# StuLiu/RegDA

Measured on AMD Instinct MI355X. Metric: src+tgt 512x512 image-pairs/sec (SSL step), higher is better.
Workload: dtype bf16; 1 GPU; st.regda.2potsdam SSL step, resnet101 DeepLabV2(PPM), batch 8+8 512x512 per GPU, online EMA teacher; global_batch=8, parallelism=dp1

## Files before the change

include/rgda_hip.h:

```cpp
#ifndef RGDA_HIP_H
#define RGDA_HIP_H

#include <stddef.h>
#include <stdint.h>

#ifdef __cplusplus
extern "C" {
#endif

#define RGDA_ABI_VERSION 10
#define RGDA_STAT_REPLICAS 8
#define RGDA_STAT_FRAC_FWD 26
#define RGDA_STAT_FRAC_BWD 40
typedef int64_t rgda_stat_t;
#define RGDA_LAYOUT_TILE 64

typedef void* rgda_stream_t;

enum rgda_status {
    RGDA_OK = 0,
    RGDA_ERR_ARG = -1,
    RGDA_ERR_WORKSPACE = -2,
    RGDA_ERR_LAUNCH = -3,
    RGDA_ERR_UNSUPPORTED = -4
// ... 237 lines not shown
int rgda_classifier_bwd(const void* hidden, int ldh, const float* w, const float* glogits,
                        void* dhidden, int lddh, float* dw, float* db, int N, int HW, int C,
                        int ncls, void* ws, size_t ws_bytes, rgda_stream_t stream);


int rgda_sumsq(const float* g, int64_t n, float* out, float* ws, rgda_stream_t stream);

int rgda_sgd_step(float* p, const float* g, float* v, float* shadow, void* p_bf16, void* shadow_bf16,
                  const float* gnorm_sq, const float* lr_dev, int64_t n, float momentum,
                  float weight_decay, float max_norm, float gscale, float ema_decay,
                  int first_step, rgda_stream_t stream);

size_t rgda_stem_wgrad_workspace(int N, int H, int W);
int rgda_stem_wgrad(const float* img, const void* dy, int lddy, float* dw, void* ws, size_t ws_bytes, int N, int H,
                    int W, int Ho, int Wo, rgda_stream_t stream);

int rgda_weight_transpose_bf16(const float* w, void* wt, int Co, int T, int Ci, rgda_stream_t stream);
int rgda_weight_transpose_batched(const int64_t* table, int n, int64_t total_blocks, rgda_stream_t stream);
int rgda_cast_bf16(const float* src, void* dst, int64_t n, rgda_stream_t stream);
int rgda_cast_f32(const void* src_bf16, float* dst, int64_t n, rgda_stream_t stream);
int rgda_ddp_accumulate_bf16(const void* recv, int world, void* out, int64_t shard_elems, rgda_stream_t stream);

typedef void* rgda_comm_t;
#define RGDA_COMM_ID_BYTES 128
#define RGDA_COMM_F32 0
#define RGDA_COMM_BF16 1
#define RGDA_COMM_I64 2
#define RGDA_COMM_F64 3
int rgda_comm_unique_id(void* id_128_bytes);
int rgda_comm_init(const void* id_128_bytes, int rank, int world, rgda_comm_t* comm);
// ... 185 lines not shown
```

regda_amd/csrc/common.h:

```cpp
#pragma once
#include <hip/hip_runtime.h>
#include <stdint.h>

#include "../../include/rgda_hip.h"

#define RGDA_CHECK_LAUNCH()                                   \
    do {                                                      \
        if (hipGetLastError() != hipSuccess) return RGDA_ERR_LAUNCH; \
    } while (0)

typedef unsigned short bf16_t;
typedef __attribute__((ext_vector_type(8))) __bf16 bf16x8;
typedef __attribute__((ext_vector_type(8))) unsigned short u16x8;
typedef __attribute__((ext_vector_type(4))) unsigned short u16x4;
typedef __attribute__((ext_vector_type(4))) short s16x4;
typedef __attribute__((ext_vector_type(16))) float f32x16;
typedef __attribute__((ext_vector_type(4))) float f32x4;

typedef __attribute__((ext_vector_type(2))) __bf16 bf16x2_t;
typedef __attribute__((ext_vector_type(2))) float f32x2_t;
static __device__ __forceinline__ float bf2f(bf16_t h) { return __uint_as_float(((unsigned)h) << 16); }
static __device__ __forceinline__ unsigned pack2bf(float lo, float hi) {
    f32x2_t v = {lo, hi};
    bf16x2_t b = __builtin_convertvector(v, bf16x2_t);
// ... 117 lines not shown
            const float unb = (b.rows_per_group > 1) ? (float)b.rows_per_group / (float)(b.rows_per_group - 1) : 1.f;
            float rm = b.rm ? b.rm[c] : 0.f, rv = b.rm ? b.rv[c] : 0.f;
            for (int g = 0; g < b.groups; ++g) {
                float gm, gv, gi;
                stat_moments(b.stats + (size_t)g * NREP * 2 * C, C, c, invM, b.eps, gm, gv, gi);
                if (b.mi) { b.mi[(size_t)g * 2 * C + c] = gm; b.mi[(size_t)g * 2 * C + C + c] = gi; }
                rm = (1.f - b.mom) * rm + b.mom * gm;
                rv = (1.f - b.mom) * rv + b.mom * gv * unb;
            }
            if (b.rm) { b.rm[c] = rm; b.rv[c] = rv; }
            if (c == 0 && b.nbt) *b.nbt += b.groups;
        }
    }
}

#include <stdlib.h>
#ifdef RGDA_TUNING
#define TUNE_ENV(name) getenv(name)
#else
#define TUNE_ENV(name) ((const char*)nullptr)
#endif
static inline hipStream_t to_stream(rgda_stream_t s) { return (hipStream_t)s; }
static inline int zero_bytes(void* p, size_t bytes, rgda_stream_t stream) {
    if (!((uintptr_t)p & 15)) return rgda_fill_zero(p, bytes, stream);
    return hipMemsetAsync(p, 0, bytes, (hipStream_t)stream) == hipSuccess ? RGDA_OK : RGDA_ERR_LAUNCH;
}
static inline int cdiv(long long a, long long b) { return (int)((a + b - 1) / b); }

#include <type_traits>
#define RGDA_MIN_CLASSES 6
// ... 17 lines not shown
```

regda_amd/csrc/conv_kernels.hip:

```cpp
#include <stdio.h>
#include <stdlib.h>
#include <string.h>

#include "common.h"
#include <type_traits>
#include <vector>

struct ConvArgs {
    const bf16_t* x;
    const bf16_t* w;
    bf16_t* y;
    const bf16_t* res;
    rgda_stat_t* stats;
    int ldx, ldy, ldres;
    int N, H, W, Cin, Ho, Wo, Cout, KH, KW, stride, pad, dil, mode;
    int M;
    int tiles_c, tiles_p;
    int rows_per_group;
    int howo_shift, wo_shift;
    unsigned long long* dbg;
    int tpw;
    int skip;
    const unsigned char* res_mask;
    const bf16_t* bn_y;
// ... 1775 lines not shown
    if (Ho != (H + 6 - 7) / 2 + 1 || Wo != (W + 6 - 7) / 2 + 1) return RGDA_ERR_ARG;
    if (Wo % 64) return RGDA_ERR_UNSUPPORTED;
    if ((long long)3 * H * W >= (1ll << 28)) return RGDA_ERR_UNSUPPORTED;
    if (((uintptr_t)ws & 15) || ws_bytes < rgda_stem_wgrad_workspace(N, H, W)) return RGDA_ERR_WORKSPACE;
    const int rpw = stem_wgrad_rows(N, Ho, Wo);
    const long long blocks = (long long)N * (Ho / rpw) * (Wo / 64);
    if (blocks > 0x7fffffffLL || (long long)N * Ho * Wo > 0x7fffffffLL) return RGDA_ERR_ARG;
    hipStream_t st = to_stream(stream);
    stem_wgrad_kernel<<<(int)blocks, 256, 0, st>>>(img, (const bf16_t*)dy, lddy, (float*)ws, H, W, Ho, Wo, rpw);
    RGDA_CHECK_LAUNCH();
    stem_wgrad_reduce_kernel<<<cdiv(64 * 147, 32), 256, 0, st>>>((const float*)ws, (int)blocks, dw);
    RGDA_CHECK_LAUNCH();
    return RGDA_OK;
}

extern "C" int rgda_stem_conv(const float* img, const void* wgt, void* y, int ldy, rgda_stat_t* stats, int stat_groups,
                              int N, int H, int W, int Ho, int Wo, rgda_stream_t stream) {
    return stem_conv_launch(img, wgt, y, ldy, stats, stat_groups, nullptr, N, H, W, Ho, Wo, stream);
}

extern "C" int rgda_stem_conv_bneval(const float* img, const void* wgt, void* y, int ldy, const float* running_mean,
                                     const float* running_var, const float* gamma, const float* beta, float eps, int relu,
                                     int N, int H, int W, int Ho, int Wo, rgda_stream_t stream) {
    BnEvalFuse e = {running_mean, running_var, gamma, beta, eps, relu};
    return stem_conv_launch(img, wgt, y, ldy, nullptr, 1, &e, N, H, W, Ho, Wo, stream);
}

struct WgradArgs {
    const bf16_t* x;
    const bf16_t* dy;
// ... 698 lines not shown
```

regda_amd/csrc/norm_kernels.hip:

```cpp
#include <stdlib.h>
#include "common.h"

struct RowLayout {
    int vpr;
    int vpb;
    int rpb;
};
static RowLayout row_layout(int C) {
    RowLayout L;
    L.vpr = C / 8;
    int v = 1;
    while (v < L.vpr && v < 256) v <<= 1;
    L.vpb = v;
    L.rpb = 256 / v;
    return L;
}

static int reduce_rows_per_block(long long M, const RowLayout& L) {
    int ny = cdiv(L.vpr, L.vpb);
    long long want = 512 / ny;
    if (const char* e = TUNE_ENV("RGDA_RED_WANT")) want = atoi(e) / ny;
    if (want < 1) want = 1;
    long long rows = (M + want - 1) / want;
    long long minrows = (long long)L.rpb * 4;
// ... 379 lines not shown
                }
                if (nscale) {
                    const float* ns = nscale + (r / rpi) * C + cg;
#pragma unroll
                    for (int e = 0; e < 8; ++e) gf[e] *= ns[e];
                }
#pragma unroll
                for (int e = 0; e < 8; ++e) { s[e] += gf[e]; q[e] += gf[e] * ((xf[e] - mean[e]) * istd[e]); }
            }
        }
    }
    rgda_stat_t* rep = sums + (size_t)((blockIdx.x + blockIdx.y * gridDim.x) & (NREP - 1)) * 2 * C;
    block_reduce_atomic(s, q, cvl, rl, vpb, rpb, cg, cok, rep, rep + C, lds, RGDA_STAT_FRAC_BWD);
}

extern "C" int rgda_bn_bwd_reduce(const void* g, int ldg, const void* y, int ldy, const uint8_t* relu_mask,
                                  const void* x, int ldx, const float* mi, const float* nscale, int rows_per_image,
                                  rgda_stat_t* sums, int64_t M, int C, int relu, const float* gamma, const float* beta,
                                  int groups, rgda_stream_t stream) {
    if (!g || !x || !mi || !sums || (relu == 1 && !y && !relu_mask) || M <= 0 || C <= 0 || (C & 7) || (ldg & 7) || (ldx & 7)) return RGDA_ERR_ARG;
    if (relu < 0 || relu > 2 || (relu == 2 && (!gamma || !beta))) return RGDA_ERR_ARG;
    if (groups < 1 || (M % groups)) return RGDA_ERR_ARG;
    hipStream_t st = to_stream(stream);
    RowLayout L = row_layout(C);
    if (L.vpb > 16) { L.vpb = 16; L.rpb = 16; }
    if (const char* e = TUNE_ENV("RGDA_RED_VPB")) { int v = atoi(e); if (v < L.vpb) { L.vpb = v; L.rpb = 256 / v; } }
    const long long Mg = M / groups;
    int rows_per_block = reduce_rows_per_block(Mg * groups, L);
    if (rows_per_block > Mg) rows_per_block = (int)((Mg + L.rpb - 1) / L.rpb * L.rpb);
    int bpg = cdiv(Mg, rows_per_block);
    dim3 grid(bpg * groups, cdiv(L.vpr, L.vpb));
    if (relu == 2)
        bn_bwd_reduce_kernel<true><<<grid, 256, 0, st>>>((const bf16_t*)g, ldg, (const bf16_t*)y, ldy, relu_mask, (const bf16_t*)x, ldx,
                                                         mi, nscale, rows_per_image, sums, Mg, C, relu, L.vpb, L.rpb,
                                                         rows_per_block, bpg, gamma, beta);
    else
        bn_bwd_reduce_kernel<false><<<grid, 256, 0, st>>>((const bf16_t*)g, ldg, (const bf16_t*)y, ldy, relu_mask, (const bf16_t*)x, ldx,
                                                          mi, nscale, rows_per_image, sums, Mg, C, relu, L.vpb, L.rpb,
                                                          rows_per_block, bpg, gamma, beta);
    RGDA_CHECK_LAUNCH();
    return RGDA_OK;
}

template <bool FROM_X>
__global__ void __launch_bounds__(256) bn_bwd_apply_kernel(const bf16_t* __restrict__ g, int ldg,
                                                           const bf16_t* __restrict__ y, int ldy,
// ... 6 lines not shown
                                                           float* dbeta, long long M, int C, int relu, int vpb, int rpb,
                                                           int rows_per_block, int bpg, const float* __restrict__ beta,
                                                           bf16_t* __restrict__ act_out, int ldact) {
    const int cvl = threadIdx.x % vpb, rl = threadIdx.x / vpb;
    const int cg = (blockIdx.y * vpb + cvl) * 8;
    const int grp = blockIdx.x / bpg, chunk = blockIdx.x % bpg;
    mi += (size_t)grp * 2 * C;
    sums += (size_t)grp * NREP * 2 * C;
    extern __shared__ __attribute__((aligned(16))) float sk_dyn[];
    const int nch = vpb * 8;
    float* const sk0 = sk_dyn;
    const float invM = 1.f / (float)M;
    for (int c = threadIdx.x; c < vpb * 8; c += 256) {
        const int cc = blockIdx.y * vpb * 8 + c;
        if (cc < C) {
            const float t1 = (float)stat_total(sums, C, cc, 0, RGDA_STAT_FRAC_BWD);
            const float t2 = (float)stat_total(sums, C, cc, 1, RGDA_STAT_FRAC_BWD);
            const float is = mi[C + cc];
            sk0[0 * nch + c] = mi[cc];
            sk0[1 * nch + c] = is;
            sk0[2 * nch + c] = gamma[cc] * is;
            sk0[3 * nch + c] = t1 * invM;
            sk0[4 * nch + c] = t2 * invM;
            if constexpr (FROM_X) {
                float fsc, fsh;
                bn_scale_shift(mi[cc], is, gamma[cc], beta[cc], fsc, fsh);
                sk0[5 * nch + c] = fsh;
            }
            if (chunk == 0 && grp == 0 && dgamma) {
                const int groups = gridDim.x / bpg;
                float dg = t2, db = t1;
                for (int g2 = 1; g2 < groups; ++g2) {
                    dg += (float)stat_total(sums + (size_t)g2 * NREP * 2 * C, C, cc, 1, RGDA_STAT_FRAC_BWD);
                    db += (float)stat_total(sums + (size_t)g2 * NREP * 2 * C, C, cc, 0, RGDA_STAT_FRAC_BWD);
                }
                atomicAdd(dgamma + cc, dg);
                atomicAdd(dbeta + cc, db);
            }
        }
    }
    __syncthreads();
    if (cg >= C) return;
    float mean[8], istd[8], k0[8], k1[8], k2[8], fsh[8];
#pragma unroll
    for (int e = 0; e < 8; ++e) {
        mean[e] = sk0[0 * nch + cvl * 8 + e];
        istd[e] = sk0[1 * nch + cvl * 8 + e];
        k0[e] = sk0[2 * nch + cvl * 8 + e];
        k1[e] = sk0[3 * nch + cvl * 8 + e];
        k2[e] = sk0[4 * nch + cvl * 8 + e];
        if constexpr (FROM_X) fsh[e] = sk0[5 * nch + cvl * 8 + e]; else fsh[e] = 0.f;
    }
// ... 37 lines not shown
                } else {
                    float yf[8];
                    cvt8(yv[u], yf);
#pragma unroll
                    for (int e = 0; e < 8; ++e) gf[e] = (yf[e] > 0.f) ? gf[e] : 0.f;
                }
            }
            if (nscale) {
                const float* ns = nscale + (r / rpi) * C + cg;
#pragma unroll
                for (int e = 0; e < 8; ++e) gf[e] *= ns[e];
            }
            if (gmask) store8(gmask + r * ldgm + cg, gf);
            float o[8];
#pragma unroll
            for (int e = 0; e < 8; ++e) o[e] = k0[e] * (gf[e] - k1[e] - (xf[e] - mean[e]) * istd[e] * k2[e]);
            store8(dx + r * lddx + cg, o);
        }
    }
}

extern "C" int rgda_bn_bwd_apply(const void* g, int ldg, const void* y, int ldy, const uint8_t* relu_mask,
                                 const void* x, int ldx,
                                 const float* mi, const float* gamma, const float* nscale, int rows_per_image,
                                 const rgda_stat_t* sums, void* dx, int lddx, void* gmask, int ldgm, float* dgamma,
                                 float* dbeta, int64_t M, int C, int relu, const float* beta, void* act_out, int ldact,
                                 int groups, rgda_stream_t stream) {
    if (!g || !x || !mi || !gamma || !sums || !dx || (relu == 1 && !y && !relu_mask) || M <= 0 || C <= 0 || (C & 7)) return RGDA_ERR_ARG;
    if (relu < 0 || relu > 2 || (relu == 2 && !beta) || (act_out && (relu != 2 || (ldact & 7) || ldact < C))) return RGDA_ERR_ARG;
    if ((ldg & 7) || (ldx & 7) || (lddx & 7) || (gmask && (ldgm & 7)) || ((dgamma == nullptr) != (dbeta == nullptr)))
        return RGDA_ERR_ARG;
// ... 1115 lines not shown
```

regda_amd/models/Encoder.py:

```python
import collections
import contextlib
import math
from typing import NamedTuple

import torch
import torch.nn as nn

from .. import ops
from .. import plan

BF = torch.bfloat16
LAYERS = {'resnet101': (3, 4, 23, 3), 'resnet50': (3, 4, 6, 3)}
POOL_SCALES = (1, 2, 3, 6)
NREP = 8
LAYOUT_TILE = 64


def _layout_blocks(co, ci, taps):
    return -(-ci // LAYOUT_TILE) * -(-co // LAYOUT_TILE) * taps

ASPP_DILATIONS = (6, 12, 18, 24)
STEM_KP = 192


# ... 168 lines not shown
WGRAD_FLUSH_AFTER = ('layer2',)


class _Unit(NamedTuple):
    x: object
    c: object
    y: object
    mi: object
    dims: tuple
    nscale: object
    rmask: object

    @property
    def on_operand_path(self):
        return self.rmask is FROM_X


class _UnitBwd:
    sums = None
    presums = None
    wgrad = None


_NO_UNIT_BWD = _UnitBwd()


class _WgradQueue:

    def __init__(self):
        self.items, self.flop, self._apart = [], 0.0, None
# ... 135 lines not shown
        self.resnet_type = rt
        self.num_classes = int(cfg['num_classes'])
        self.device = torch.device('cuda', torch.cuda.current_device())
        self._build_params()
        self._init_weights()
        self._anchor = torch.zeros(1, device=self.device, requires_grad=True)
        self._drop_override = None
        self.wgrad_group_gflop = 500.0
        self.relu_sign_mask = 1
        self.factored_ppm = True
        self.group_small_convs = True
        self.small_bn = True
        self.bn_on_operand = True
        self.bn_operand_units = {'stem', 'bn1', 'bn2'}
        self.bn_operand_level = 2
        self._head_stream = None
        self._mat_cache = {}
        self._synced_version = -1
        self.sync_weights()

    def _build_params(self):
        dev = self.device
        entries, self.blocks, self._head_first = _param_entries(self.resnet_type, self.head_kind, self.num_classes)

        n_param = sum(_pad64(math.prod(s)) for _, k, s in entries if k in ('convw', 'vec'))
        n_buf = sum(_pad64(math.prod(s)) for _, k, s in entries if k == 'buf')
        n_nbt = sum(1 for _, k, _s in entries if k == 'nbt')
        self.flat_p = torch.zeros(n_param, device=dev)
        self.flat_g = torch.zeros(n_param, device=dev)
        self.flat_pb = torch.zeros(n_param, dtype=BF, device=dev)
# ... 576 lines not shown
                                     1, dx_res, csums, G, ce.y if (crelu == 1 and cmask is None) else None, ce.c, ce.mi, crelu,
                                     ce.nscale, cHo * cWo, relu_mask=cmask, res_mask=dx_res_mask,
                                     bn_gamma=None if cbn is None else cbn.gamma, bn_beta=None if cbn is None else cbn.beta)
                    T['unit_bwd'][ckey].sums = csums
                    fused = True
                except ValueError:
                    T['unit_bwd'][ckey].presums = csums
            if not fused:
                if conv_queue is not None:
                    conv_queue.append((dc, conv.wtb, dx, N, Ho, Wo, H, W, conv.k, conv.k, conv.stride, conv.pad, conv.dil, 1,
                                       dx_res, None, 1, dx_res_mask))
                else:
                    ops.conv2d(dc, conv.wtb, dx, N, Ho, Wo, H, W, conv.k, conv.k, conv.stride, conv.pad, conv.dil, 1,
                               dx_res, None, res_mask=dx_res_mask)
        return dx, gm

    def _stem_fwd(self, T, xs, Ng, H, W, H1, W1, main_stream):
        dev = self.device
        bn = self.bns['encoder.resnet.bn1']
        G = len(xs)
        N, M = Ng * G, Ng * G * H1 * W1
        y = torch.empty(M, 64, dtype=BF, device=dev)
        if T is None:
            for gi, xg in enumerate(xs):
                ops.stem_conv_bneval(xg, self.stem_wb, y[gi * Ng * H1 * W1:(gi + 1) * Ng * H1 * W1], bn.rm, bn.rv, bn.gamma,
                                     bn.beta, True, Ng, H, W, H1, W1)
            return y, None
        side = self._side_stream()
        plan.wait_event(side, plan.record_event(main_stream))
        with ops.use_stream(side):
# ... 290 lines not shown
        hh, ww = h, w
        for bi in range(len(self.blocks) - 1, -1, -1):
            p, inpl, planes, stride, dil, ds = self.blocks[bi]
            if dbg is not None:
                dbg[p] = _nchw(g, N, hh, ww)
                hh, ww = hh * stride, ww * stride
            below = (self.blocks[bi - 1][0] + '.3', True) if bi > 0 else None
            g = self._block_bwd(T, self.blocks[bi], g, below)
            self._progress(T, self._offset_of(p + '.conv1'))
            if bi > 0 and T['wgrads'].items:
                stage = p.split('.')[-2]
                if stage in WGRAD_FLUSH_AFTER and self.blocks[bi - 1][0].split('.')[-2] != stage:
                    self._flush_wgrads(T)
        self._flush_wgrads(T)
        idx, (N, H1, W1, H2, W2) = T['pool']
        ga0 = torch.empty(N * H1 * W1, 64, dtype=BF, device=dev)
        ops.maxpool_bwd(g, idx, ga0, N, H1, W1, 64, H2, W2)
        self._cbr_bwd(T, 'stem', C['encoder.resnet.conv1'], B['encoder.resnet.bn1'], ga0, True, stem=True)
        self._flush_wgrads(T)
        if T.get('mark') is not None:
            T['mark']('backward main chain done')
        if T.get('wgrad_stream') is not None:
            plan.wait_stream(T['main_stream'], T['wgrad_stream'])

    def attach_grads(self):
        for name, par in self._views.items():
            par.grad = self._gviews[name]

    def _prepare_grads(self):
        if any(par.grad is None for par in self._views.values()):
            self.flat_g.zero_()
            self.attach_grads()

# ... 52 lines not shown
```

regda_amd/ops.py:

```python
import ctypes

import torch

from ._lib import lib


MIN_CLASSES, MAX_CLASSES = 6, 16


def check_class_count(c, who='class_num'):
    if not MIN_CLASSES <= int(c) <= MAX_CLASSES:
        raise ValueError(f'{who}: {c} classes; the kernels serve {MIN_CLASSES} <= class_num <= {MAX_CLASSES}')


_LDS_LOSS_ROW, _LDS_PCL, _LDS_REFINE = 0, 1, 2


def check_step_shape(c, k, H, W, who='step'):
    check_class_count(c, who)
    L = lib()
    w = (int(W) + 15) // 16
    row, lim = L.size('rgda_class_lds', _LDS_LOSS_ROW, c, w, W), L.size('rgda_class_lds_limit', _LDS_LOSS_ROW)
    if row > lim:
        raise ValueError(f'{who}: {c} classes at {W}-pixel rows need {row} B of LDS in the fused upsample + loss row pass, '
# ... 667 lines not shown


def stem_conv_bneval(img, wb, y, rm, rv, gamma, beta, relu, N, H, W, Ho, Wo, eps=1e-5):
    lib().call('rgda_stem_conv_bneval', img.data_ptr(), wb.data_ptr(), y.data_ptr(), _ld(y), rm.data_ptr(), rv.data_ptr(),
               gamma.data_ptr(), beta.data_ptr(), eps, int(relu), N, H, W, Ho, Wo, _stream())


def stem_im2col(img, col, N, H, W, Ho, Wo):
    lib().call('rgda_stem_im2col', img.data_ptr(), col.data_ptr(), N, H, W, Ho, Wo, col.shape[1], _stream())


_STEM_WS = {}
_STEM_WS_OLD = []


def stem_wgrad(img, dy, dw, N, H, W, Ho, Wo):
    assert dw.is_contiguous() and dw.dtype == torch.float32 and dw.numel() == 64 * 147 and img.is_contiguous()
    L = lib()
    nbytes = L.size('rgda_stem_wgrad_workspace', N, H, W)
    if nbytes == 0:
        raise ValueError('rgda_stem_wgrad: geometry not served (Wo % 64 != 0): use stem_im2col + conv2d_wgrad')
    key = (img.device.index, _stream())
    ws = _STEM_WS.get(key)
    if ws is None or ws.numel() < nbytes:
        if ws is not None:
            _STEM_WS_OLD.append(ws)
        ws = torch.empty(nbytes, dtype=torch.uint8, device=img.device)
        _STEM_WS[key] = ws
    L.call('rgda_stem_wgrad', img.data_ptr(), dy.data_ptr(), _ld(dy), dw.data_ptr(), ws.data_ptr(), ws.numel(), N, H, W, Ho, Wo,
           _stream())


def bn_stats(x, stats, M, C):
    lib().call('rgda_bn_stats', x.data_ptr(), _ld(x), _stat(stats), M, C, _stream())


def bn_finalize(stats, mi, rm, rv, nbt, M, C, eps=1e-5, momentum=0.1, groups=1):
    lib().call('rgda_bn_finalize', _stat(stats), mi.data_ptr(), _p(rm), _p(rv), _p(nbt), M, C, groups, eps, momentum,
               _stream())


def bn_apply(x, mi, gamma, beta, y, M, C, relu, res=None, nscale=None, rows_per_image=0, groups=1):
    lib().call('rgda_bn_apply', x.data_ptr(), _ld(x), mi.data_ptr(), gamma.data_ptr(), beta.data_ptr(), _p(res),
               _ld(res) if res is not None else 0, _p(nscale), rows_per_image, y.data_ptr(), _ld(y), M, C,
               int(relu), groups, _stream())
# ... 1005 lines not shown
```

Measured before the change: 448.0 pairs/s.

## Fuse stem maxpool backward, BN backward and weight-gradient into two kernels

Replaces the stem backward chain (maxpool_bwd into a full-resolution gradient tensor, then BN/ReLU backward and stem wgrad) with two passes. The first reduces BN backward sums straight from the pooled gradient and argmax indices. The second recomputes the unpooled, ReLU-masked BN input gradient on the fly inside the stem wgrad MFMA kernel. This avoids materialising and re-reading the largest activation gradient in the network, at the cost of redoing the pool-gradient scatter twice and a more complex kernel.

```diff
diff --git a/include/rgda_hip.h b/include/rgda_hip.h
--- a/include/rgda_hip.h
+++ b/include/rgda_hip.h
@@ -275,6 +275,14 @@
 size_t rgda_stem_wgrad_workspace(int N, int H, int W);
 int rgda_stem_wgrad(const float* img, const void* dy, int lddy, float* dw, void* ws, size_t ws_bytes, int N, int H,
                     int W, int Ho, int Wo, rgda_stream_t stream);
+
+int rgda_stem_bwd_sums(const void* gy, const uint8_t* idx, const void* x, int ldx, const float* mi, const float* gamma,
+                       const float* beta, rgda_stat_t* sums, int N, int H1, int W1, int Hp, int Wp, int groups,
+                       rgda_stream_t stream);
+int rgda_stem_wgrad_bn(const float* img, const void* x, int ldx, const void* gy, const uint8_t* idx,
+                       const rgda_stat_t* sums, const float* mi, const float* gamma, const float* beta, float* dgamma,
+                       float* dbeta, int groups, int group, float* dw, void* ws, size_t ws_bytes, int N, int H, int W,
+                       int H1, int W1, int Hp, int Wp, rgda_stream_t stream);
 
 int rgda_weight_transpose_bf16(const float* w, void* wt, int Co, int T, int Ci, rgda_stream_t stream);
 int rgda_weight_transpose_batched(const int64_t* table, int n, int64_t total_blocks, rgda_stream_t stream);
diff --git a/regda_amd/csrc/common.h b/regda_amd/csrc/common.h
--- a/regda_amd/csrc/common.h
+++ b/regda_amd/csrc/common.h
@@ -155,6 +155,86 @@
     }
 }
 
+struct BnBwdConsts {
+    float mean, istd, k0, k1, k2, fsh;
+    float t1, t2;
+};
+static __device__ __forceinline__ BnBwdConsts bn_bwd_consts(const rgda_stat_t* __restrict__ sums, const float* __restrict__ mi,
+                                                            const float* __restrict__ gamma, const float* __restrict__ beta,
+                                                            int C, int cc, float invM, bool from_x) {
+    BnBwdConsts k;
+    k.t1 = (float)stat_total(sums, C, cc, 0, RGDA_STAT_FRAC_BWD);
+    k.t2 = (float)stat_total(sums, C, cc, 1, RGDA_STAT_FRAC_BWD);
+    k.mean = mi[cc];
+    k.istd = mi[C + cc];
+    k.k0 = gamma[cc] * k.istd;
+    k.k1 = k.t1 * invM;
+    k.k2 = k.t2 * invM;
+    k.fsh = 0.f;
+    if (from_x) {
+        float fsc;
+        bn_scale_shift(k.mean, k.istd, gamma[cc], beta[cc], fsc, k.fsh);
+    }
+    return k;
+}
+static __device__ __forceinline__ void bn_bwd_param_grads(const rgda_stat_t* __restrict__ sums, int C, int cc, int groups,
+                                                          float t1, float t2, float* dgamma, float* dbeta) {
+    float dg = t2, db = t1;
+    for (int g2 = 1; g2 < groups; ++g2) {
+        dg += (float)stat_total(sums + (size_t)g2 * NREP * 2 * C, C, cc, 1, RGDA_STAT_FRAC_BWD);
+        db += (float)stat_total(sums + (size_t)g2 * NREP * 2 * C, C, cc, 0, RGDA_STAT_FRAC_BWD);
+    }
+    atomicAdd(dgamma + cc, dg);
+    atomicAdd(dbeta + cc, db);
+}
+static __device__ __forceinline__ float bn_bwd_dx(float g, float x, float mean, float istd, float k0, float k1, float k2) {
+    return k0 * (g - k1 - (x - mean) * istd * k2);
+}
+
+struct PoolGrad8 {
+    uint4 g[4];
+    uint2 ix[4];
+    unsigned tap[4];
+};
+static __device__ __forceinline__ void pool_grad_load(const bf16_t* __restrict__ gy, const uint8_t* __restrict__ idx, int n,
+                                                      int hi, int wi, int Ho, int Wo, int C, int c0, PoolGrad8& p) {
+    const int ho = hi >> 1, wo = wi >> 1;
+    const int w0 = (n * Ho + ho) * Wo + wo;
+    const bool row1 = (hi & 1) && ho + 1 < Ho, col1 = (wi & 1) && wo + 1 < Wo;
+    const unsigned kh = (unsigned)(hi & 1) + 1u, kw = (unsigned)(wi & 1) + 1u;
+#pragma unroll
+    for (int s = 0; s < 4; ++s) {
+        const bool ok = ((s & 2) == 0 || row1) && ((s & 1) == 0 || col1);
+        p.tap[s] = ok ? ((s & 2) ? 0u : kh * 3u) + ((s & 1) ? 0u : kw) : 0xffu;
+        if (ok) {
+            const unsigned o = (unsigned)(w0 + ((s & 2) ? Wo : 0) + (s & 1)) * (unsigned)C + (unsigned)c0;
+            p.ix[s] = *(const uint2*)(idx + o);
+            p.g[s] = *(const uint4*)((const unsigned char*)gy + 2u * o);
+        }
+    }
+}
+static __device__ __forceinline__ void pool_grad_sum(const PoolGrad8& p, float (&acc)[8]) {
+#pragma unroll
+    for (int e = 0; e < 8; ++e) acc[e] = 0.f;
+#pragma unroll
+    for (int s = 0; s < 4; ++s) {
+        if (p.tap[s] == 0xffu) continue;
+        const unsigned gw[4] = {p.g[s].x, p.g[s].y, p.g[s].z, p.g[s].w};
+#pragma unroll
+        for (int e = 0; e < 8; ++e) {
+            const unsigned b = ((e < 4 ? p.ix[s].x : p.ix[s].y) >> (8 * (e & 3))) & 0xffu;
+            const float g = __uint_as_float((e & 1) ? (gw[e >> 1] & 0xffff0000u) : (gw[e >> 1] << 16));
+            if (b == p.tap[s]) acc[e] += g;
+        }
+    }
+#pragma unroll
+    for (int e = 0; e < 8; e += 2) {
+        const unsigned r = pack2bf(acc[e], acc[e + 1]);
+        acc[e] = __uint_as_float(r << 16);
+        acc[e + 1] = __uint_as_float(r & 0xffff0000u);
+    }
+}
+
 #include <stdlib.h>
 #ifdef RGDA_TUNING
 #define TUNE_ENV(name) getenv(name)
diff --git a/regda_amd/csrc/conv_kernels.hip b/regda_amd/csrc/conv_kernels.hip
--- a/regda_amd/csrc/conv_kernels.hip
+++ b/regda_amd/csrc/conv_kernels.hip
@@ -1813,6 +1813,246 @@
     return RGDA_OK;
 }
 
+__global__ void __launch_bounds__(256) stem_wgrad_bn_kernel(const float* __restrict__ img, const bf16_t* __restrict__ x, int ldx,
+                                                            const bf16_t* __restrict__ gy, const uint8_t* __restrict__ idx,
+                                                            const rgda_stat_t* __restrict__ sums, const float* __restrict__ mi,
+                                                            const float* __restrict__ gamma, const float* __restrict__ beta,
+                                                            float* dgamma, float* dbeta, int groups, int group, long long M,
+                                                            float* __restrict__ part, int H, int W, int Ho, int Wo, int Hp,
+                                                            int Wp, int rpw) {
+#if defined(__HIP_DEVICE_COMPILE__)
+    constexpr int BP = 64, KP = 192;
+    constexpr int SWP = 136, SROW = SWP * 8, NSLOT = 9;
+    constexpr int DT = 64 * 128;
+    __shared__ __attribute__((aligned(256))) unsigned char smem[2 * DT + NSLOT * SROW];
+    __shared__ __attribute__((aligned(16))) float ktab[6][64];
+    unsigned char* const sd = smem;
+    unsigned char* const srow = smem + 2 * DT;
+
+    const int t = threadIdx.x, lane = t & 63;
+    const int wave = __builtin_amdgcn_readfirstlane(t >> 6);
+    const int wi = wave & 1, wj = wave >> 1;
+    const int wtiles = Wo / BP, rblocks = Ho / rpw;
+    const int wo0 = (blockIdx.x % wtiles) * BP;
+    const int ho0 = ((blockIdx.x / wtiles) % rblocks) * rpw, n = blockIdx.x / (wtiles * rblocks);
+    const int hbase = ho0 * 2 - 3;
+
+    if (t < 64) {
+        const rgda_stat_t* gs = sums + (size_t)group * NREP * 2 * 64;
+        const float invM = 1.f / (float)M;
+        const BnBwdConsts k = bn_bwd_consts(gs, mi + (size_t)group * 2 * 64, gamma, beta, 64, t, invM, true);
+        ktab[0][t] = k.mean; ktab[1][t] = k.istd; ktab[2][t] = k.k0;
+        ktab[3][t] = k.k1; ktab[4][t] = k.k2; ktab[5][t] = k.fsh;
+        if (blockIdx.x == 0 && dgamma) bn_bwd_param_grads(gs, 64, t, groups, k.t1, k.t2, dgamma, dbeta);
+    }
+    __syncthreads();
+
+    const size_t plane = (size_t)H * W;
+    const float* const img_n = img + (size_t)n * 3 * plane;
+    auto load_px = [&](int j, int x_, float (&v)[3]) {
+        const int hi = hbase + j, wcol = wo0 * 2 - 3 + x_;
+        const bool ok = (unsigned)hi < (unsigned)H && (unsigned)wcol < (unsigned)W && x_ < 134;
+        const size_t o = (size_t)(ok ? hi : 0) * W + (ok ? wcol : 0);
+#pragma unroll
+        for (int c = 0; c < 3; ++c) v[c] = ok ? img_n[c * plane + o] : 0.f;
+    };
+    auto store_px = [&](int j, int x_, const float (&v)[3]) {
+        uint2 p;
+        p.x = pack2bf(v[0], v[1]);
+        p.y = pack2bf(v[2], 0.f);
+        *(uint2*)(srow + (j % NSLOT) * SROW + x_ * 8) = p;
+    };
+    const int doct = t & 7, dpx = t >> 3, dq = (wo0 >> 1) + dpx;
+    struct DyLoad {
+        uint4 x[2];
+        uint4 g[4];
+        uint2 ix[4];
+        int ho;
+    };
+    const bool col1 = dq + 1 < Wp;
+    auto load_dy = [&](int ho, DyLoad& d) {
+        d.ho = ho;
+        const unsigned xo = ((unsigned)((n * Ho + ho) * Wo + wo0 + 2 * dpx) * (unsigned)ldx + (unsigned)(doct * 8)) * 2u;
+        d.x[0] = *(const uint4*)((const unsigned char*)x + xo);
+        d.x[1] = *(const uint4*)((const unsigned char*)x + (xo + 2u * (unsigned)ldx));
+        const bool rowb = (ho & 1) && (ho >> 1) + 1 < Hp;
+        const int w0 = (n * Hp + (ho >> 1)) * Wp + dq;
+#pragma unroll
+        for (int s = 0; s < 4; ++s) {
+            if (((s & 2) == 0 || rowb) && ((s & 1) == 0 || col1)) {
+                const unsigned o = (unsigned)(w0 + ((s & 2) ? Wp : 0) + (s & 1)) * 64u + (unsigned)(doct * 8);
+                d.ix[s] = *(const uint2*)(idx + o);
+                d.g[s] = *(const uint4*)((const unsigned char*)gy + 2u * o);
+            }
+        }
+    };
+    auto store_dy = [&](int buf, const DyLoad& d) {
+        const bool rowb = (d.ho & 1) && (d.ho >> 1) + 1 < Hp;
+        const unsigned ta = (unsigned)(((d.ho & 1) + 1) * 3);
+        float gf[2][8], o[2][8];
+#pragma unroll
+        for (int h = 0; h < 2; ++h) {
+            PoolGrad8 pg;
+#pragma unroll
+            for (int s = 0; s < 4; ++s) { pg.g[s] = d.g[s]; pg.ix[s] = d.ix[s]; }
+            if (h == 0) {
+                pg.tap[0] = ta + 1; pg.tap[1] = 0xffu; pg.tap[2] = rowb ? 1u : 0xffu; pg.tap[3] = 0xffu;
+            } else {
+                pg.tap[0] = ta + 2; pg.tap[1] = col1 ? ta : 0xffu;
+                pg.tap[2] = rowb ? 2u : 0xffu; pg.tap[3] = (rowb && col1) ? 0u : 0xffu;
+            }
+            pool_grad_sum(pg, gf[h]);
+        }
+#pragma unroll
+        for (int e4 = 0; e4 < 8; e4 += 4) {
+            const f32x4 kmean = *(const f32x4*)&ktab[0][doct * 8 + e4], kistd = *(const f32x4*)&ktab[1][doct * 8 + e4];
+            const f32x4 k0 = *(const f32x4*)&ktab[2][doct * 8 + e4], k1 = *(const f32x4*)&ktab[3][doct * 8 + e4];
+            const f32x4 k2 = *(const f32x4*)&ktab[4][doct * 8 + e4], kfsh = *(const f32x4*)&ktab[5][doct * 8 + e4];
+#pragma unroll
+            for (int h = 0; h < 2; ++h) {
+                const unsigned xw[4] = {d.x[h].x, d.x[h].y, d.x[h].z, d.x[h].w};
+#pragma unroll
+                for (int j = 0; j < 4; ++j) {
+                    const int e = e4 + j;
+                    const float xf = __uint_as_float((e & 1) ? (xw[e >> 1] & 0xffff0000u) : (xw[e >> 1] << 16));
+                    const float g = (bn_affine(xf, k0[j], kfsh[j]) > 0.f) ? gf[h][e] : 0.f;
+                    o[h][e] = bn_bwd_dx(g, xf, kmean[j], kistd[j], k0[j], k1[j], k2[j]);
+                }
+            }
+        }
+#pragma unroll
+        for (int h = 0; h < 2; ++h) {
+            uint4 v;
+            v.x = pack2bf(o[h][0], o[h][1]); v.y = pack2bf(o[h][2], o[h][3]);
+            v.z = pack2bf(o[h][4], o[h][5]); v.w = pack2bf(o[h][6], o[h][7]);
+            const int p = 2 * dpx + h, f = (p >> 1) & 1;
+            *(uint4*)(sd + buf * DT + p * 128 + ((((doct >> 2) ^ f) << 6) | ((doct & 3) << 4))) = v;
+        }
+    };
+#pragma unroll
+    for (int i = 0; i < 4; ++i) {
+        const int ii = t + 256 * i;
+        if (ii < 7 * SWP) {
+            float v[3];
+            load_px(ii / SWP, ii % SWP, v);
+            store_px(ii / SWP, ii % SWP, v);
+        }
+    }
+    DyLoad dyl;
+    load_dy(ho0, dyl);
+    store_dy(0, dyl);
+    const int nj0 = t / SWP, nx0 = t % SWP;
+    const int nj1 = (t + 256) / SWP, nx1 = (t + 256) % SWP;
+    const bool second = t + 256 < 2 * SWP;
+    float na0[3] = {0.f, 0.f, 0.f}, na1[3] = {0.f, 0.f, 0.f}, nb0[3] = {0.f, 0.f, 0.f}, nb1[3] = {0.f, 0.f, 0.f};
+    if (1 < rpw) {
+        load_px(7 + nj0, nx0, na0);
+        if (second) load_px(7 + nj1, nx1, na1);
+    }
+    const int g = lane >> 4, la = lane & 15;
+    const int krow = (g >> 1) * 8 + (la >> 2);
+    const int kcol2 = ((g & 1) * 16 + (la & 3) * 4) * 2;
+    auto pack_tr = [](s16x4 lo, s16x4 hi) {
+        u16x8 v8 = {(bf16_t)lo[0], (bf16_t)lo[1], (bf16_t)lo[2], (bf16_t)lo[3],
+                    (bf16_t)hi[0], (bf16_t)hi[1], (bf16_t)hi[2], (bf16_t)hi[3]};
+        return __builtin_bit_cast(bf16x8, v8);
+    };
+    auto tr_dy = [&](const unsigned char* base, int byte, int r0) {
+        const int r1 = r0 + 4;
+        const unsigned char* p0 = base + r0 * 128 + ((((byte >> 6) ^ ((r0 >> 1) & 1)) << 6) | (byte & 63));
+        const unsigned char* p1 = base + r1 * 128 + ((((byte >> 6) ^ ((r1 >> 1) & 1)) << 6) | (byte & 63));
+        return pack_tr(__builtin_amdgcn_ds_read_tr16_b64_v4i16((s16x4 __attribute__((address_space(3)))*)(p0)),
+                       __builtin_amdgcn_ds_read_tr16_b64_v4i16((s16x4 __attribute__((address_space(3)))*)(p1)));
+    };
+    auto tr_img = [&](const unsigned char* rowbase, int r0) {
+        const unsigned char* p0 = rowbase + r0 * 16 + kcol2;
+        return pack_tr(__builtin_amdgcn_ds_read_tr16_b64_v4i16((s16x4 __attribute__((address_space(3)))*)(p0)),
+                       __builtin_amdgcn_ds_read_tr16_b64_v4i16((s16x4 __attribute__((address_space(3)))*)(p0 + 64)));
+    };
+    f32x16 acc[4];
+#pragma unroll
+    for (int j = 0; j < 4; ++j)
+#pragma unroll
+        for (int e = 0; e < 16; ++e) acc[j][e] = 0.f;
+    const int kh0 = wj * 4, nkh = wj ? 3 : 4;
+
+    for (int r = 0; r < rpw; ++r) {
+        asm volatile("s_waitcnt lgkmcnt(0)" ::: "memory");
+        __builtin_amdgcn_s_barrier();
+        if (r + 1 < rpw) load_dy(ho0 + r + 1, dyl);
+        if (r + 2 < rpw) {
+            load_px(2 * r + 9 + nj0, nx0, nb0);
+            if (second) load_px(2 * r + 9 + nj1, nx1, nb1);
+        }
+        const unsigned char* sdc = sd + (r & 1) * DT;
+        const int s0 = (2 * r + kh0) % NSLOT;
+#pragma unroll
+        for (int kk = 0; kk < 4; ++kk) {
+            const int r0 = kk * 16 + krow;
+            const bf16x8 af = tr_dy(sdc, wi * 64 + kcol2, r0);
+#pragma unroll
+            for (int a = 0; a < 4; ++a) {
+                if (a < nkh) {
+                    const int slot = (s0 + a >= NSLOT) ? s0 + a - NSLOT : s0 + a;
+                    const bf16x8 bf = tr_img(srow + slot * SROW, r0);
+                    acc[a] = __builtin_amdgcn_mfma_f32_32x32x16_bf16(af, bf, acc[a], 0, 0, 0);
+                }
+            }
+        }
+        if (r + 1 < rpw) {
+            store_dy((r + 1) & 1, dyl);
+            store_px(2 * r + 7 + nj0, nx0, na0);
+            if (second) store_px(2 * r + 7 + nj1, nx1, na1);
+        }
+#pragma unroll
+        for (int c = 0; c < 3; ++c) { na0[c] = nb0[c]; na1[c] = nb1[c]; }
+    }
+    float* out = part + (size_t)blockIdx.x * 64 * KP;
+    const int lrow = lane & 31, lk = lane >> 5;
+    const int kw = lrow >> 2, c = lrow & 3;
+    if (kw < 7 && c < 3) {
+#pragma unroll
+        for (int a = 0; a < 4; ++a)
+            if (a < nkh) {
+                const int k = ((kh0 + a) * 7 + kw) * 3 + c;
+#pragma unroll
+                for (int g4 = 0; g4 < 4; ++g4)
+#pragma unroll
+                    for (int e = 0; e < 4; ++e)
+                        out[(wi * 32 + 8 * g4 + 4 * lk + e) * KP + k] = acc[a][4 * g4 + e];
+            }
+    }
+#endif
+}
+
+extern "C" int rgda_stem_wgrad_bn(const float* img, const void* x, int ldx, const void* gy, const uint8_t* idx,
+                                  const rgda_stat_t* sums, const float* mi, const float* gamma, const float* beta,
+                                  float* dgamma, float* dbeta, int groups, int group, float* dw, void* ws, size_t ws_bytes,
+                                  int N, int H, int W, int Ho, int Wo, int Hp, int Wp, rgda_stream_t stream) {
+    if (!img || !x || !gy || !idx || !sums || !mi || !gamma || !beta || !dw || !ws || N <= 0 || H <= 0 || W <= 0 || (ldx & 7) ||
+        ldx < 64)
+        return RGDA_ERR_ARG;
+    if (groups < 1 || group < 0 || group >= groups || (dgamma == nullptr) != (dbeta == nullptr)) return RGDA_ERR_ARG;
+    if (Ho != (H + 6 - 7) / 2 + 1 || Wo != (W + 6 - 7) / 2 + 1) return RGDA_ERR_ARG;
+    if (Hp != (Ho + 2 - 3) / 2 + 1 || Wp != (Wo + 2 - 3) / 2 + 1) return RGDA_ERR_ARG;
+    if (Wo % 64) return RGDA_ERR_UNSUPPORTED;
+    if ((long long)3 * H * W >= (1ll << 28)) return RGDA_ERR_UNSUPPORTED;
+    if (((uintptr_t)ws & 15) || ws_bytes < rgda_stem_wgrad_workspace(N, H, W)) return RGDA_ERR_WORKSPACE;
+    const int rpw = stem_wgrad_rows(N, Ho, Wo);
+    const long long blocks = (long long)N * (Ho / rpw) * (Wo / 64);
+    if (blocks > 0x7fffffffLL || (long long)N * Ho * Wo > 0x7fffffffLL) return RGDA_ERR_ARG;
+    if ((long long)N * Ho * Wo * ldx * 2 >= (1ll << 32)) return RGDA_ERR_UNSUPPORTED;
+    hipStream_t st = to_stream(stream);
+    stem_wgrad_bn_kernel<<<(int)blocks, 256, 0, st>>>(img, (const bf16_t*)x, ldx, (const bf16_t*)gy, idx, sums, mi, gamma, beta,
+                                                      group == 0 ? dgamma : nullptr, group == 0 ? dbeta : nullptr, groups, group,
+                                                      (long long)N * Ho * Wo, (float*)ws, H, W, Ho, Wo, Hp, Wp,
+                                                      rpw);
+    RGDA_CHECK_LAUNCH();
+    stem_wgrad_reduce_kernel<<<cdiv(64 * 147, 32), 256, 0, st>>>((const float*)ws, (int)blocks, dw);
+    RGDA_CHECK_LAUNCH();
+    return RGDA_OK;
+}
+
 extern "C" int rgda_stem_conv(const float* img, const void* wgt, void* y, int ldy, rgda_stat_t* stats, int stat_groups,
                               int N, int H, int W, int Ho, int Wo, rgda_stream_t stream) {
     return stem_conv_launch(img, wgt, y, ldy, stats, stat_groups, nullptr, N, H, W, Ho, Wo, stream);
diff --git a/regda_amd/csrc/norm_kernels.hip b/regda_amd/csrc/norm_kernels.hip
--- a/regda_amd/csrc/norm_kernels.hip
+++ b/regda_amd/csrc/norm_kernels.hip
@@ -417,6 +417,95 @@
     block_reduce_atomic(s, q, cvl, rl, vpb, rpb, cg, cok, rep, rep + C, lds, RGDA_STAT_FRAC_BWD);
 }
 
+static void bwd_reduce_grid(long long Mg, int C, int groups, RowLayout& L, int& rows_per_block, int& bpg, dim3& grid) {
+    L = row_layout(C);
+    if (L.vpb > 16) { L.vpb = 16; L.rpb = 16; }
+    if (const char* e = TUNE_ENV("RGDA_RED_VPB")) { int v = atoi(e); if (v < L.vpb) { L.vpb = v; L.rpb = 256 / v; } }
+    rows_per_block = reduce_rows_per_block(Mg * groups, L);
+    if (rows_per_block > Mg) rows_per_block = (int)((Mg + L.rpb - 1) / L.rpb * L.rpb);
+    bpg = cdiv(Mg, rows_per_block);
+    grid = dim3(bpg * groups, cdiv(L.vpr, L.vpb));
+}
+
+__global__ void __launch_bounds__(256) stem_bwd_sums_kernel(const bf16_t* __restrict__ gy, const uint8_t* __restrict__ idx,
+                                                            const bf16_t* __restrict__ x, int ldx,
+                                                            const float* __restrict__ mi, rgda_stat_t* sums, long long M, int C,
+                                                            int H, int W, int Ho, int Wo, int vpb, int rpb, int rows_per_block,
+                                                            int bpg, const float* __restrict__ gamma,
+                                                            const float* __restrict__ beta) {
+    constexpr int RB = 2;
+    __shared__ float lds[256 * 16];
+    const int cvl = threadIdx.x % vpb;
+    int rl = threadIdx.x / vpb;
+    if (vpb == 8) rl = 2 * (((rl >> 3) & 1) * 8 + (rl & 7)) + (rl >> 4);
+    const int cg = (blockIdx.y * vpb + cvl) * 8;
+    const bool cok = cg < C;
+    const int grp = blockIdx.x / bpg, chunk = blockIdx.x % bpg;
+    mi += (size_t)grp * 2 * C;
+    sums += (size_t)grp * NREP * 2 * C;
+    float s[8] = {0}, q[8] = {0};
+    if (cok) {
+        float mean[8], istd[8], fsc[8], fsh[8];
+#pragma unroll
+        for (int e = 0; e < 8; ++e) {
+            mean[e] = mi[cg + e]; istd[e] = mi[C + cg + e];
+            bn_scale_shift(mean[e], istd[e], gamma[cg + e], beta[cg + e], fsc[e], fsh[e]);
+        }
+        const int r0 = (int)((long long)grp * M + (long long)chunk * rows_per_block);
+        const int r1 = (int)min((long long)(grp + 1) * M, (long long)r0 + rows_per_block);
+        int wi = (r0 + rl) % W, hi = ((r0 + rl) / W) % H, n = (r0 + rl) / (W * H);
+        const bf16_t* xp = x + (size_t)(r0 + rl) * ldx + cg;
+        const size_t xstep = (size_t)rpb * ldx;
+        for (int rb = r0 + rl; rb < r1; rb += rpb * RB) {
+            u16x8 xv[RB];
+            PoolGrad8 pg[RB];
+#pragma unroll
+            for (int u = 0; u < RB; ++u) {
+                if (rb + u * rpb < r1) {
+                    xv[u] = *(const u16x8*)xp;
+                    pool_grad_load(gy, idx, n, hi, wi, Ho, Wo, C, cg, pg[u]);
+                }
+                xp += xstep;
+                wi += rpb;
+                while (wi >= W) { wi -= W; if (++hi == H) { hi = 0; ++n; } }
+            }
+#pragma unroll
+            for (int u = 0; u < RB; ++u) {
+                if (rb + u * rpb >= r1) break;
+                float gf[8], xf[8];
+                pool_grad_sum(pg[u], gf);
+                cvt8(xv[u], xf);
+#pragma unroll
+                for (int e = 0; e < 8; ++e) gf[e] = (bn_affine(xf[e], fsc[e], fsh[e]) > 0.f) ? gf[e] : 0.f;
+#pragma unroll
+                for (int e = 0; e < 8; ++e) { s[e] += gf[e]; q[e] += gf[e] * ((xf[e] - mean[e]) * istd[e]); }
+            }
+        }
+    }
+    const unsigned wg = blockIdx.y * gridDim.x + blockIdx.x;
+    rgda_stat_t* rep = sums + (size_t)(wg & (NREP - 1)) * 2 * C;
+    block_reduce_atomic(s, q, cvl, rl, vpb, rpb, cg, cok, rep, rep + C, lds, RGDA_STAT_FRAC_BWD);
+}
+
+extern "C" int rgda_stem_bwd_sums(const void* gy, const uint8_t* idx, const void* x, int ldx, const float* mi,
+                                  const float* gamma, const float* beta, rgda_stat_t* sums, int N, int H, int W, int Ho,
+                                  int Wo, int groups, rgda_stream_t stream) {
+    if (!gy || !idx || !x || !mi || !gamma || !beta || !sums || N <= 0 || H <= 0 || W <= 0 || (ldx & 7) || ldx < 64)
+        return RGDA_ERR_ARG;
+    if (Ho != (H + 2 - 3) / 2 + 1 || Wo != (W + 2 - 3) / 2 + 1) return RGDA_ERR_ARG;
+    if (groups < 1 || (N % groups)) return RGDA_ERR_ARG;
+    if (W % 64) return RGDA_ERR_UNSUPPORTED;
+    if ((long long)N * H * W > 0x7fffffffLL - (1 << 20)) return RGDA_ERR_ARG;
+    if ((long long)N * Ho * Wo * 64 * 2 >= (1ll << 32)) return RGDA_ERR_UNSUPPORTED;
+    RowLayout L; int rows_per_block, bpg; dim3 grid;
+    const long long Mg = (long long)N * H * W / groups;
+    bwd_reduce_grid(Mg, 64, groups, L, rows_per_block, bpg, grid);
+    stem_bwd_sums_kernel<<<grid, 256, 0, to_stream(stream)>>>((const bf16_t*)gy, idx, (const bf16_t*)x, ldx, mi, sums, Mg, 64, H, W,
+                                                             Ho, Wo, L.vpb, L.rpb, rows_per_block, bpg, gamma, beta);
+    RGDA_CHECK_LAUNCH();
+    return RGDA_OK;
+}
+
 extern "C" int rgda_bn_bwd_reduce(const void* g, int ldg, const void* y, int ldy, const uint8_t* relu_mask,
                                   const void* x, int ldx, const float* mi, const float* nscale, int rows_per_image,
                                   rgda_stat_t* sums, int64_t M, int C, int relu, const float* gamma, const float* beta,
@@ -425,14 +514,9 @@
     if (relu < 0 || relu > 2 || (relu == 2 && (!gamma || !beta))) return RGDA_ERR_ARG;
     if (groups < 1 || (M % groups)) return RGDA_ERR_ARG;
     hipStream_t st = to_stream(stream);
-    RowLayout L = row_layout(C);
-    if (L.vpb > 16) { L.vpb = 16; L.rpb = 16; }
-    if (const char* e = TUNE_ENV("RGDA_RED_VPB")) { int v = atoi(e); if (v < L.vpb) { L.vpb = v; L.rpb = 256 / v; } }
+    RowLayout L; int rows_per_block, bpg; dim3 grid;
     const long long Mg = M / groups;
-    int rows_per_block = reduce_rows_per_block(Mg * groups, L);
-    if (rows_per_block > Mg) rows_per_block = (int)((Mg + L.rpb - 1) / L.rpb * L.rpb);
-    int bpg = cdiv(Mg, rows_per_block);
-    dim3 grid(bpg * groups, cdiv(L.vpr, L.vpb));
+    bwd_reduce_grid(Mg, C, groups, L, rows_per_block, bpg, grid);
     if (relu == 2)
         bn_bwd_reduce_kernel<true><<<grid, 256, 0, st>>>((const bf16_t*)g, ldg, (const bf16_t*)y, ldy, relu_mask, (const bf16_t*)x, ldx,
                                                          mi, nscale, rows_per_image, sums, Mg, C, relu, L.vpb, L.rpb,
@@ -469,28 +553,15 @@
     for (int c = threadIdx.x; c < vpb * 8; c += 256) {
         const int cc = blockIdx.y * vpb * 8 + c;
         if (cc < C) {
-            const float t1 = (float)stat_total(sums, C, cc, 0, RGDA_STAT_FRAC_BWD);
-            const float t2 = (float)stat_total(sums, C, cc, 1, RGDA_STAT_FRAC_BWD);
-            const float is = mi[C + cc];
-            sk0[0 * nch + c] = mi[cc];
-            sk0[1 * nch + c] = is;
-            sk0[2 * nch + c] = gamma[cc] * is;
-            sk0[3 * nch + c] = t1 * invM;
-            sk0[4 * nch + c] = t2 * invM;
-            if constexpr (FROM_X) {
-                float fsc, fsh;
-                bn_scale_shift(mi[cc], is, gamma[cc], beta[cc], fsc, fsh);
-                sk0[5 * nch + c] = fsh;
-            }
+            const BnBwdConsts k = bn_bwd_consts(sums, mi, gamma, beta, C, cc, invM, FROM_X);
+            sk0[0 * nch + c] = k.mean;
+            sk0[1 * nch + c] = k.istd;
+            sk0[2 * nch + c] = k.k0;
+            sk0[3 * nch + c] = k.k1;
+            sk0[4 * nch + c] = k.k2;
+            if constexpr (FROM_X) sk0[5 * nch + c] = k.fsh;
             if (chunk == 0 && grp == 0 && dgamma) {
-                const int groups = gridDim.x / bpg;
-                float dg = t2, db = t1;
-                for (int g2 = 1; g2 < groups; ++g2) {
-                    dg += (float)stat_total(sums + (size_t)g2 * NREP * 2 * C, C, cc, 1, RGDA_STAT_FRAC_BWD);
-                    db += (float)stat_total(sums + (size_t)g2 * NREP * 2 * C, C, cc, 0, RGDA_STAT_FRAC_BWD);
-                }
-                atomicAdd(dgamma + cc, dg);
-                atomicAdd(dbeta + cc, db);
+                bn_bwd_param_grads(sums, C, cc, gridDim.x / bpg, k.t1, k.t2, dgamma, dbeta);
             }
         }
     }
@@ -558,7 +629,7 @@
             if (gmask) store8(gmask + r * ldgm + cg, gf);
             float o[8];
 #pragma unroll
-            for (int e = 0; e < 8; ++e) o[e] = k0[e] * (gf[e] - k1[e] - (xf[e] - mean[e]) * istd[e] * k2[e]);
+            for (int e = 0; e < 8; ++e) o[e] = bn_bwd_dx(gf[e], xf[e], mean[e], istd[e], k0[e], k1[e], k2[e]);
             store8(dx + r * lddx + cg, o);
         }
     }
diff --git a/regda_amd/models/Encoder.py b/regda_amd/models/Encoder.py
--- a/regda_amd/models/Encoder.py
+++ b/regda_amd/models/Encoder.py
@@ -206,6 +206,17 @@
     @property
     def on_operand_path(self):
         return self.rmask is FROM_X
+
+
+def stem_bwd_fused_ok(unit, g, enabled=True, debug_taps=None, debug_grads=None):
+    if not enabled or debug_taps is not None or debug_grads is not None:
+        return False
+    if not (isinstance(unit.x, tuple) and unit.on_operand_path and unit.y is None and unit.mi is not None):
+        return False
+    N, H, W, H1, W1 = unit.dims
+    if N % len(unit.x) or not ops.stem_bwd_fused_served(H, W, N):
+        return False
+    return g.dim() == 2 and g.shape[1] == 64 and g.is_contiguous()
 
 
 class _UnitBwd:
@@ -371,6 +382,7 @@
         self.bn_on_operand = True
         self.bn_operand_units = {'stem', 'bn1', 'bn2'}
         self.bn_operand_level = 2
+        self.fuse_stem_bwd = True
         self._head_stream = None
         self._mat_cache = {}
         self._synced_version = -1
@@ -977,6 +989,20 @@
                     ops.conv2d(dc, conv.wtb, dx, N, Ho, Wo, H, W, conv.k, conv.k, conv.stride, conv.pad, conv.dil, 1,
                                dx_res, None, res_mask=dx_res_mask)
         return dx, gm
+
+    def _stem_bwd_fused(self, T, g, idx, H2, W2):
+        e = T['stem']
+        conv, bn = self.convs['encoder.resnet.conv1'], self.bns['encoder.resnet.bn1']
+        N, H, W, H1, W1 = e.dims
+        G = len(e.x)
+        Ng = N // G
+        sums = T['sums_pool'].take(G * NREP * 2 * 64)
+        ops.stem_bwd_sums(g, idx, e.c, e.mi, bn.gamma, bn.beta, sums, N, H1, W1, H2, W2, groups=G)
+        rows, prow = Ng * H1 * W1, Ng * H2 * W2
+        for gi, xg in enumerate(e.x):
+            ops.stem_wgrad_bn(xg, e.c[gi * rows:(gi + 1) * rows], g[gi * prow:(gi + 1) * prow], idx[gi * prow:(gi + 1) * prow],
+                              sums, e.mi, bn.gamma, bn.beta, bn.dgamma, bn.dbeta, G, gi, conv.g.view(64, 147), Ng, H, W, H1, W1,
+                              H2, W2)
 
     def _stem_fwd(self, T, xs, Ng, H, W, H1, W1, main_stream):
         dev = self.device
@@ -1297,9 +1323,12 @@
                     self._flush_wgrads(T)
         self._flush_wgrads(T)
         idx, (N, H1, W1, H2, W2) = T['pool']
-        ga0 = torch.empty(N * H1 * W1, 64, dtype=BF, device=dev)
-        ops.maxpool_bwd(g, idx, ga0, N, H1, W1, 64, H2, W2)
-        self._cbr_bwd(T, 'stem', C['encoder.resnet.conv1'], B['encoder.resnet.bn1'], ga0, True, stem=True)
+        if stem_bwd_fused_ok(T['stem'], g, self.fuse_stem_bwd, getattr(self, '_debug_taps', None), dbg):
+            self._stem_bwd_fused(T, g, idx, H2, W2)
+        else:
+            ga0 = torch.empty(N * H1 * W1, 64, dtype=BF, device=dev)
+            ops.maxpool_bwd(g, idx, ga0, N, H1, W1, 64, H2, W2)
+            self._cbr_bwd(T, 'stem', C['encoder.resnet.conv1'], B['encoder.resnet.bn1'], ga0, True, stem=True)
         self._flush_wgrads(T)
         if T.get('mark') is not None:
             T['mark']('backward main chain done')
diff --git a/regda_amd/ops.py b/regda_amd/ops.py
--- a/regda_amd/ops.py
+++ b/regda_amd/ops.py
@@ -705,12 +705,7 @@
 _STEM_WS_OLD = []
 
 
-def stem_wgrad(img, dy, dw, N, H, W, Ho, Wo):
-    assert dw.is_contiguous() and dw.dtype == torch.float32 and dw.numel() == 64 * 147 and img.is_contiguous()
-    L = lib()
-    nbytes = L.size('rgda_stem_wgrad_workspace', N, H, W)
-    if nbytes == 0:
-        raise ValueError('rgda_stem_wgrad: geometry not served (Wo % 64 != 0): use stem_im2col + conv2d_wgrad')
+def _stem_workspace(img, nbytes):
     key = (img.device.index, _stream())
     ws = _STEM_WS.get(key)
     if ws is None or ws.numel() < nbytes:
@@ -718,8 +713,45 @@
             _STEM_WS_OLD.append(ws)
         ws = torch.empty(nbytes, dtype=torch.uint8, device=img.device)
         _STEM_WS[key] = ws
-    L.call('rgda_stem_wgrad', img.data_ptr(), dy.data_ptr(), _ld(dy), dw.data_ptr(), ws.data_ptr(), ws.numel(), N, H, W, Ho, Wo,
-           _stream())
+    return ws.data_ptr(), ws.numel()
+
+
+def stem_wgrad(img, dy, dw, N, H, W, Ho, Wo):
+    assert dw.is_contiguous() and dw.dtype == torch.float32 and dw.numel() == 64 * 147 and img.is_contiguous()
+    L = lib()
+    nbytes = L.size('rgda_stem_wgrad_workspace', N, H, W)
+    if nbytes == 0:
+        raise ValueError('rgda_stem_wgrad: geometry not served (Wo % 64 != 0): use stem_im2col + conv2d_wgrad')
+    L.call('rgda_stem_wgrad', img.data_ptr(), dy.data_ptr(), _ld(dy), dw.data_ptr(), *_stem_workspace(img, nbytes), N, H, W,
+           Ho, Wo, _stream())
+
+
+def stem_bwd_fused_served(H, W, N=1):
+    H1, W1 = (H + 6 - 7) // 2 + 1, (W + 6 - 7) // 2 + 1
+    return H > 0 and W > 0 and N > 0 and W1 % 64 == 0 and 3 * H * W < (1 << 28) and N * H1 * W1 * 64 * 2 < (1 << 32)
+
+
+def _pooled_contiguous(gy, idx):
+    if not (gy.is_contiguous() and idx.is_contiguous() and gy.shape[-1] == 64 and idx.shape[-1] == 64):
+        raise ValueError('stem backward: the pooled gradient and the argmax taps must be contiguous [rows, 64] tensors')
+
+
+def stem_bwd_sums(gy, idx, x, mi, gamma, beta, sums, N, H1, W1, Hp, Wp, groups=1):
+    _pooled_contiguous(gy, idx)
+    lib().call('rgda_stem_bwd_sums', gy.data_ptr(), idx.data_ptr(), x.data_ptr(), _ld(x), mi.data_ptr(), gamma.data_ptr(),
+               beta.data_ptr(), _stat(sums), N, H1, W1, Hp, Wp, groups, _stream())
+
+
+def stem_wgrad_bn(img, x, gy, idx, sums, mi, gamma, beta, dgamma, dbeta, groups, group, dw, N, H, W, H1, W1, Hp, Wp):
+    assert dw.is_contiguous() and dw.dtype == torch.float32 and dw.numel() == 64 * 147 and img.is_contiguous()
+    _pooled_contiguous(gy, idx)
+    L = lib()
+    nbytes = L.size('rgda_stem_wgrad_workspace', N, H, W)
+    if nbytes == 0:
+        raise ValueError('rgda_stem_wgrad_bn: geometry not served (W1 % 64 != 0): use the unfused chain')
+    L.call('rgda_stem_wgrad_bn', img.data_ptr(), x.data_ptr(), _ld(x), gy.data_ptr(), idx.data_ptr(), _stat(sums),
+           mi.data_ptr(), gamma.data_ptr(), beta.data_ptr(), _p(dgamma), _p(dbeta), groups, group, dw.data_ptr(),
+           *_stem_workspace(img, nbytes), N, H, W, H1, W1, Hp, Wp, _stream())
 
 
 def bn_stats(x, stats, M, C):
```

Result: no change. 449.2 pairs/s, median of 6 (+0.3%).
